# akanimax/thr3ed_atom

Measured on AMD Instinct MI355X. Metric: ray-samples/sec (fwd+bwd) training step, 800x800 images @ 128^3 SH-2 ReLU field, higher is better.
Workload: dtype f32

## Files before the change

thr3ed_atom_amd/csrc/relu_field_kernels.hip:

```cpp
#include <hip/hip_runtime.h>
#include <stdint.h>

#include <atomic>
#include <climits>
#include <cmath>
#include <cstdlib>
#include <type_traits>

#include "relu_field.h"

namespace {

#ifndef RF_FWD_WAVES
#define RF_FWD_WAVES 4
#endif
#ifndef RF_EMIT_WAVES
#define RF_EMIT_WAVES 6
#endif
#ifndef RF_EMIT_G
#define RF_EMIT_G 2
#endif
constexpr int kWave = 64;
constexpr int kWavesPerBlock = 4;
constexpr int kBlock = kWave * kWavesPerBlock;
// ... 1868 lines not shown
  {
    const int4* __restrict__ h4 = reinterpret_cast<const int4*>(hist);
    const int n4 = seg0 >> 2;
    int k4 = t;
    for (; k4 + 3 * 1024 < n4; k4 += 4 * 1024) {
      const int4 a0 = h4[k4], a1 = h4[k4 + 1024], a2 = h4[k4 + 2048], a3 = h4[k4 + 3072];
      front += (a0.x + a0.y) + (a0.z + a0.w) + (a1.x + a1.y) + (a1.z + a1.w) + (a2.x + a2.y) + (a2.z + a2.w) + (a3.x + a3.y) + (a3.z + a3.w);
    }
    for (; k4 < n4; k4 += 1024) {
      const int4 a0 = h4[k4];
      front += (a0.x + a0.y) + (a0.z + a0.w);
    }
  }
#pragma unroll
  for (int d = 1; d < kWave; d <<= 1) front += __shfl_xor(front, d);
  const int k = seg0 + t;
  const int c = k < nkeys ? hist[k] : 0;
  int incl = c;
#pragma unroll
  for (int d = 1; d < kWave; d <<= 1) {
    const int up = __shfl_up(incl, d);
    if (lane >= d) incl += up;
  }
  if (lane == kWave - 1) {
    s_front[wave] = front;
    s_own[wave] = incl;
  }
  __syncthreads();
  int base = 0, before = 0, own = 0;
#pragma unroll
  for (int w = 0; w < 16; ++w) {
    base += s_front[w];
    if (w < wave) before += s_own[w];
    own += s_own[w];
  }
  if (k < nkeys) {
    const int excl = base + before + incl - c;
    offsets[k] = excl;
    cursor[k] = excl;
  }
  if (t == 0 && seg0 + 1024 >= nkeys) offsets[nkeys] = base + own;
}

__global__ __launch_bounds__(1024) void bin_offsets_kernel(BinLists lists, int nkeys) { bin_offsets_body(lists, nkeys, blockIdx.y, blockIdx.x); }

template <int Q>
__global__ __launch_bounds__(256) void scatter_records_kernel(const short* __restrict__ keys, const float4* __restrict__ rec,
                                                              long long capacity, int* __restrict__ cursor,
                                                              float4* __restrict__ out, int* __restrict__ hist, int nkeys) {
  constexpr int NCH = 4;
  __shared__ long long s_slot[4][NCH * kWave];
  __shared__ int s_pos[4][NCH * kWave];
  const int lane = threadIdx.x & (kWave - 1), wave = threadIdx.x >> 6;
  if (hist)
    for (long long k = (long long)blockIdx.x * blockDim.x + threadIdx.x; k < nkeys; k += (long long)gridDim.x * blockDim.x) hist[k] = 0;
  const long long slot0 = ((long long)blockIdx.x * 4 + wave) * (NCH * kWave);
  if (slot0 >= capacity) return;
  int key[NCH], run[NCH], hl[NCH], base[NCH];
  bool head[NCH];
  unsigned long long act[NCH];
#pragma unroll
  for (int i = 0; i < NCH; ++i) {
    const long long slot = slot0 + i * kWave + lane;
    key[i] = slot < capacity ? (int)keys[slot] : -1;
  }
#pragma unroll
  for (int i = 0; i < NCH; ++i) {
    const bool active = key[i] >= 0;
    act[i] = __ballot(active);
    const int prev = __shfl_up(key[i], 1);
    head[i] = active && (lane == 0 || prev != key[i]);
    const unsigned long long heads = __ballot(head[i]);
    const unsigned long long ends = __ballot(head[i] || !active);
    const unsigned long long above = (lane == 63) ? 0ull : (ends & ~((2ull << lane) - 1ull));
    run[i] = (above ? __builtin_ctzll(above) : 64) - lane;
    const unsigned long long below = heads & ((lane == 63) ? ~0ull : ((2ull << lane) - 1ull));
    hl[i] = below ? 63 - __builtin_clzll(below) : 0;
  }
#pragma unroll
  for (int i = 0; i < NCH; ++i) base[i] = head[i] ? atomicAdd(&cursor[key[i]], run[i]) : 0;
  int n_act = 0;
#pragma unroll
  for (int i = 0; i < NCH; ++i) {
    const int pos = __shfl(base[i], hl[i]) + (lane - hl[i]);
    if (key[i] >= 0) {
      const int e = n_act + __popcll(act[i] & ((1ull << lane) - 1ull));
      s_slot[wave][e] = slot0 + i * kWave + lane;
      s_pos[wave][e] = pos;
    }
    n_act += __popcll(act[i]);
  }
  wave_lds_fence();
  const int items = n_act * Q;
  for (int it = lane; it < items; it += kWave) {
    const int e = it / Q, part = it - e * Q;
    out[(long long)s_pos[wave][e] * Q + part] = rec[s_slot[wave][e] * Q + part];
  }
}

constexpr int kBrickThreads = 512;

__host__ __device__ inline int brick_node_stride(int C) { return (C + 3) / 4 * 4; }
__host__ __device__ inline int brick_row_stride(int B, int C) {
  const int row = B * brick_node_stride(C);
  return row + ((48 - row % 64) + 64) % 64;
}
__host__ __device__ inline int brick_slab_stride(int B, int C) {
  const int slab = B * brick_row_stride(B, C);
  return slab + ((8 - slab % 64) + 64) % 64;
}
__host__ __device__ inline int brick_acc_words(int B, int C) { return B * brick_slab_stride(B, C) + 64; }

#ifdef RF_BRICK_PROFILE
__device__ unsigned long long g_brick_prof[8];
#define RF_PROF_MARK(slot)                                                       \
  do {                                                                           \
    const unsigned long long now_ = __builtin_readcyclecounter();                \
    prof_acc_[slot] += now_ - prof_t_;                                           \
    prof_t_ = now_;                                                              \
  } while (0)
#define RF_PROF_START()                                              \
  unsigned long long prof_acc_[8] = {0, 0, 0, 0, 0, 0, 0, 0};        \
  unsigned long long prof_t_ = __builtin_readcyclecounter()
#define RF_PROF_END()                                                            \
  do {                                                                           \
    if (threadIdx.x == 0) {                                                      \
      _Pragma("unroll") for (int s_ = 0; s_ < 8; ++s_)                           \
        if (prof_acc_[s_]) atomicAdd(&g_brick_prof[s_], prof_acc_[s_]);          \
    }                                                                            \
  } while (0)
#else
#define RF_PROF_MARK(slot) do { } while (0)
#define RF_PROF_START() do { } while (0)
#define RF_PROF_END() do { } while (0)
#endif

__device__ __forceinline__ void brick_range_entry(const BrickArgs& a, const long long* __restrict__ offsets, int bx, int by, int bz, int e,
                                                  int& start, int& cnt) {
  const int ex = e / 5, eyz = e - ex * 5;
  const int ox = ex == 2, xf = ex >= 1;
  const int oy = (0x16 >> eyz) & 1, oz = (0x18 >> eyz) & 1;
  const int f0 = (0x32310 >> (4 * eyz)) & 7, f1 = (0x33313 >> (4 * eyz)) & 7;
  const int sx = bx - ox, sy = by - oy, sz = bz - oz;
  start = 0;
  cnt = 0;
  if (sx >= 0 && sy >= 0 && sz >= 0) {
    const long long* off = offsets + ((long long)((((sx << 1) | xf) * a.nby + sy) * a.nbz + sz) << 2);
    const long long rs = off[f0];
    start = (int)rs;
    cnt = (int)(off[f1 + 1] - rs);
  }
}

template <int K, bool ADAM, bool ONE_ROUND, int TH = kBrickThreads, int BX = 8, bool MIRROR = false>
__device__ __forceinline__ void brick_flush(const GridArgs& g, const BrickArgs& a, const float* acc, bool any, int X0, int Y0, int Z0,
                                            float* gdens, float* gfeat) {
  static_assert(!MIRROR || (ADAM && ONE_ROUND && BX == 4), "the mirror write-out rides on the one-round optimizer flush of 4 x 8 x 8 bricks");
  constexpr int C = 3 * K + 1;
  constexpr int CS = (C + 3) / 4 * 4;
  const int B = ONE_ROUND ? 8 : (1 << a.shift);
  const int SY = brick_row_stride(B, C), SX = brick_slab_stride(B, C);
  const int tid = threadIdx.x;
  const bool split = g.layout == RF_LAYOUT_SPLIT;
  if (split && (C & 3) == 0 && (g.dstride & 3) == 0 && (C == 4 || (g.fstride & 3) == 0)) {
    constexpr int QN = C / 4;
    constexpr int QR = QN > 1 ? QN - 1 : 1;
    const int nq = (BX == 4 ? 4 : B) * B * B * QN;
    auto quad_of = [&](int i, int& fx, int& fy, int& fz, int& qd) -> bool {
      const int col = (i >> a.shift) / QN, r = i - col * (B * QN);
      const bool first = r < B;
      fz = first ? r : (r - B) / QR;
      qd = first ? 0 : 1 + (r - B) - fz * QR;
      fx = col >> a.shift;
      fy = col & (B - 1);
      return i < nq && X0 + fx < g.X && Y0 + fy < g.Y && Z0 + fz < g.Z;
    };
    if constexpr (ADAM) {
      constexpr int U = (QN == 7) ? 4 : 1;
      const AdamArgs& ad = a.adam;
      if constexpr (ONE_ROUND) {
        unsigned int bo[QN];
        int lds_at[QN];
        float4 p4[QN];
        vf4 m4[QN], v4[QN];
#pragma unroll
        for (int u = 0; u < QN; ++u) {
          int fx, fy, fz, qd;
          if (u == 0) {
            fx = tid >> 6;
            fy = (tid >> 3) & 7;
            fz = tid & 7;
            qd = 0;
          } else {
            const int j = (u - 1) * TH + tid, col = j / 48, r = j - col * 48;
            fz = r / 6;
            qd = 1 + r - 6 * fz;
            fx = col >> 3;
            fy = col & 7;
          }
          const bool ok = X0 + fx < g.X && Y0 + fy < g.Y && Z0 + fz < g.Z;
          const unsigned int lin = ok ? node_lin(g, X0 + fx, Y0 + fy, Z0 + fz) : 0u;
          const unsigned int o = u == 0 ? __umul24(lin, (unsigned)g.dstride) : __umul24(lin, (unsigned)g.fstride) + 4u * (unsigned)(qd - 1);
          bo[u] = ok ? o * 4u : 0xffffffffu;
          lds_at[u] = fx * SX + fy * SY + fz * CS + 4 * qd;
        }
#pragma unroll
        for (int u = 0; u < QN; ++u) {
          if (bo[u] != 0xffffffffu) {
            const char* pb = reinterpret_cast<const char*>(u == 0 ? ad.p1 : ad.p2);
            const char* mb = reinterpret_cast<const char*>(u == 0 ? ad.m1 : ad.m2);
            const char* vb = reinterpret_cast<const char*>(u == 0 ? ad.v1 : ad.v2);
            p4[u] = *reinterpret_cast<const float4*>(pb + bo[u]);
            m4[u] = __builtin_nontemporal_load(reinterpret_cast<const vf4*>(mb + bo[u]));
            v4[u] = __builtin_nontemporal_load(reinterpret_cast<const vf4*>(vb + bo[u]));
          }
        }
#pragma unroll
        for (int u = 0; u < QN; ++u) {
          if (bo[u] == 0xffffffffu) continue;
          const float4 gq = any ? *reinterpret_cast<const float4*>(&acc[lds_at[u]]) : make_float4(0.f, 0.f, 0.f, 0.f);
          float gg[4] = {gq.x, gq.y, gq.z, gq.w};
          float pn[4] = {p4[u].x, p4[u].y, p4[u].z, p4[u].w};
          if (u == 0 && g.mode == RF_DENSITY_ABS) {
            const float dv = pn[0] * g.rho;
            gg[0] = (dv > 0.f) ? gg[0] : ((dv < 0.f) ? -gg[0] : 0.0f);
          }
          vf4 mn, vn;
#pragma unroll
          for (int c = 0; c < 4; ++c) {
            float mm = m4[u][c], vv = v4[u][c];
            adam_update(pn[c], mm, vv, gg[c], ad.step, ad.b1, ad.b2, ad.eps, ad.inv_bc2_sqrt);
            mn[c] = mm;
            vn[c] = vv;
          }
          char* pb = reinterpret_cast<char*>(u == 0 ? ad.p1 : ad.p2);
          char* mb = reinterpret_cast<char*>(u == 0 ? ad.m1 : ad.m2);
          char* vb = reinterpret_cast<char*>(u == 0 ? ad.v1 : ad.v2);
          *reinterpret_cast<float4*>(pb + bo[u]) = make_float4(pn[0], pn[1], pn[2], pn[3]);
          __builtin_nontemporal_store(mn, reinterpret_cast<vf4*>(mb + bo[u]));
          __builtin_nontemporal_store(vn, reinterpret_cast<vf4*>(vb + bo[u]));
          if constexpr (MIRROR) *reinterpret_cast<float4*>(const_cast<float*>(&acc[lds_at[u]])) = make_float4(pn[0], pn[1], pn[2], pn[3]);
        }
        if constexpr (MIRROR) {
          __syncthreads();
          constexpr int F = 3 * K, FQ = 2 * F, CQ = FQ + 2;
          for (int i = tid; i < 32 * CQ; i += TH) {
            const int col = i / CQ, r = i - col * CQ;
            const int fx = col >> 3, fy = col & 7;
            const float* img = acc + fx * SX + fy * SY;
            const unsigned int lin0 = node_lin(g, X0 + fx, Y0 + fy, Z0);
            float v[4];
            if (r < FQ) {
#pragma unroll
              for (int t = 0; t < 4; ++t) {
                const int e = 4 * r + t;
                const int nz = e / F, f = e - nz * F;
                const int colour = f / K, k = f - colour * K;
                v[t] = img[nz * CS + (k == 0 ? 1 + colour : 4 + colour * (K - 1) + (k - 1))];
              }
              *reinterpret_cast<float4*>(gfeat + (size_t)(__umul24(lin0, (unsigned)F) + 4u * (unsigned)r)) = make_float4(v[0], v[1], v[2], v[3]);
            } else {
              const int z0 = 4 * (r - FQ);
#pragma unroll
              for (int t = 0; t < 4; ++t) v[t] = img[(z0 + t) * CS];
              *reinterpret_cast<float4*>(gdens + (size_t)(lin0 + (unsigned)z0)) = make_float4(v[0], v[1], v[2], v[3]);
            }
          }
        }
        return;
      } else {
      for (int i0 = tid; i0 < nq; i0 += TH * U) {
        unsigned int off[U];
        float4 p4[U];
        vf4 m4[U], v4[U];
#pragma unroll
        for (int u = 0; u < U; ++u) {
          int fx, fy, fz, qd;
          const bool ok = quad_of(i0 + u * TH, fx, fy, fz, qd);
          const unsigned int lin = ok ? node_lin(g, X0 + fx, Y0 + fy, Z0 + fz) : 0u;
          const unsigned int o = qd == 0 ? lin * (unsigned)g.dstride : (lin * (unsigned)g.fstride + 4u * (unsigned)(qd - 1)) | 0x80000000u;
          off[u] = ok ? o : 0xffffffffu;
        }
#pragma unroll
        for (int u = 0; u < U; ++u) {
          if (off[u] != 0xffffffffu) {
            const bool rest = off[u] >> 31;
            const unsigned int o = off[u] & 0x7fffffffu;
#ifdef RF_BRICK_PROFILE
            if (a.stagger & 0x10000) { p4[u] = make_float4(0.f, 0.f, 0.f, 0.f); m4[u] = vf4{0.f, 0.f, 0.f, 0.f}; v4[u] = vf4{1.f, 1.f, 1.f, 1.f}; continue; }
#endif
            p4[u] = *reinterpret_cast<const float4*>((rest ? ad.p2 : ad.p1) + o);
            m4[u] = __builtin_nontemporal_load(reinterpret_cast<const vf4*>((rest ? ad.m2 : ad.m1) + o));
            v4[u] = __builtin_nontemporal_load(reinterpret_cast<const vf4*>((rest ? ad.v2 : ad.v1) + o));
          }
        }
#pragma unroll
        for (int u = 0; u < U; ++u) {
          if (off[u] == 0xffffffffu) continue;
          const bool rest = off[u] >> 31;
          const unsigned int o = off[u] & 0x7fffffffu;
          int fx, fy, fz, qd;
          quad_of(i0 + u * TH, fx, fy, fz, qd);
          const float4 gq = any ? *reinterpret_cast<const float4*>(&acc[fx * SX + fy * SY + fz * CS + 4 * qd]) : make_float4(0.f, 0.f, 0.f, 0.f);
          float gg[4] = {gq.x, gq.y, gq.z, gq.w};
          float pn[4] = {p4[u].x, p4[u].y, p4[u].z, p4[u].w};
          if (!rest && g.mode == RF_DENSITY_ABS) {
// ... 21 lines not shown
          __builtin_nontemporal_store(mn, reinterpret_cast<vf4*>((rest ? ad.m2 : ad.m1) + o));
          __builtin_nontemporal_store(vn, reinterpret_cast<vf4*>((rest ? ad.v2 : ad.v1) + o));
        }
      }
      }
      return;
    }
    for (int i = tid; i < nq; i += TH) {
      int fx, fy, fz, qd;
      if (!quad_of(i, fx, fy, fz, qd)) continue;
      const long long lin = node_lin(g, X0 + fx, Y0 + fy, Z0 + fz);
      float4 v = any ? *reinterpret_cast<const float4*>(&acc[fx * SX + fy * SY + fz * CS + 4 * qd]) : make_float4(0.f, 0.f, 0.f, 0.f);
      if (qd == 0 && g.mode == RF_DENSITY_ABS) {
        const float dv = g.dens[lin * g.dstride] * g.rho;
        v.x = (dv > 0.f) ? v.x : ((dv < 0.f) ? -v.x : 0.0f);
      }
      const long long off = (qd == 0) ? lin * g.dstride : lin * g.fstride + 4 * (qd - 1);
      if (qd == 0) {
        float4* dst = reinterpret_cast<float4*>(gdens + off);
        if (a.accumulate) {
          const float4 o = *dst;
          v = make_float4(o.x + v.x, o.y + v.y, o.z + v.z, o.w + v.w);
        }
        *dst = v;
      } else {
        float4* dst = reinterpret_cast<float4*>(gfeat + off);
        if (a.accumulate) {
          const float4 o = *dst;
          v = make_float4(o.x + v.x, o.y + v.y, o.z + v.z, o.w + v.w);
        }
        const vf4 v4 = {v.x, v.y, v.z, v.w};
        __builtin_nontemporal_store(v4, reinterpret_cast<vf4*>(dst));
      }
    }
    return;
  }
  const int n_first = split ? 4 : 1;
  const int n_second = C - n_first;
  for (int pass = 0; pass < 2; ++pass) {
    const int nch = pass == 0 ? n_first : n_second;
    if (nch == 0) continue;
    const int run = B * nch;
    float* out = pass == 0 ? gdens : gfeat;
    const long long ostride = pass == 0 ? g.dstride : g.fstride;
    for (int i = tid; i < (BX == 4 ? 4 : B) * B * run; i += TH) {
      const int col = i / run, r = i - col * run;
      const int fz = r / nch, c2 = r - fz * nch;
      const int fx = col >> a.shift, fy = col & (B - 1);
      const int X = X0 + fx, Y = Y0 + fy, Z = Z0 + fz;
      if (X >= g.X || Y >= g.Y || Z >= g.Z) continue;
      int lds_c;
      if (split) {
        lds_c = pass * 4 + c2;
      } else if (pass == 0) {
        lds_c = 0;
      } else {
        const int col3 = c2 / K, kk = c2 - col3 * K;
        lds_c = (kk == 0) ? 1 + col3 : 4 + col3 * (K - 1) + (kk - 1);
      }
      const long long lin = node_lin(g, X, Y, Z);
      float v = any ? acc[fx * SX + fy * SY + fz * CS + lds_c] : 0.0f;
      if (lds_c == 0 && g.mode == RF_DENSITY_ABS) {
        const float dv = g.dens[lin * g.dstride] * g.rho;
        v = (dv > 0.f) ? v : ((dv < 0.f) ? -v : 0.0f);
      }
      float* dst = out + lin * ostride + (long long)c2 * (pass == 1 && !split ? a.fmul : 1);
      *dst = a.accumulate ? (*dst + v) : v;
    }
  }
}

__device__ __forceinline__ uint32_t lds_offset(const void* p) { return (uint32_t)(uintptr_t)p; }
template <int OFF>
__device__ __forceinline__ void lds_request_f32(float& v, uint32_t addr) {
  asm volatile("ds_read_b32 %0, %1 offset:%2" : "+v"(v) : "v"(addr), "n"(OFF));
}
__device__ __forceinline__ void lds_request_u8(uint32_t& v, uint32_t addr) {
  asm volatile("ds_read_u8 %0, %1" : "+v"(v) : "v"(addr));
}
__device__ __forceinline__ void lds_wait(uint32_t& a, uint32_t& b) { asm volatile("s_waitcnt lgkmcnt(0)" : "+v"(a), "+v"(b)); }
__device__ __forceinline__ void lds_wait(float& a, float& b, float& c, float& d, uint32_t& f) {
  asm volatile("s_waitcnt lgkmcnt(0)" : "+v"(a), "+v"(b), "+v"(c), "+v"(d), "+v"(f));
}
__device__ __forceinline__ void lds_wait(float& a, float& b, float& c, float& d, float& e, uint32_t& f) {
  asm volatile("s_waitcnt lgkmcnt(0)" : "+v"(a), "+v"(b), "+v"(c), "+v"(d), "+v"(e), "+v"(f));
}
__device__ __forceinline__ void lds_wait(float& a, float& b, float& c, float& d, float& e, float& e2, float& e3, uint32_t& f) {
  asm volatile("s_waitcnt lgkmcnt(0)" : "+v"(a), "+v"(b), "+v"(c), "+v"(d), "+v"(e), "+v"(e2), "+v"(e3), "+v"(f));
}

constexpr int kGatherBatch = 256;
constexpr int kGatherWtab = 24;
__host__ __device__ constexpr int gather_record_words(int C4) { return C4 + 8; }
typedef float f32x4 __attribute__((ext_vector_type(4)));

__host__ __device__ inline int gather_lds_words(int B, int C, int BX = 8) {
  const int C4 = (C + 3) / 4 * 4;
  const int gb = BX == 4 ? kGatherBatch / 2 : kGatherBatch;
  const int batch = gb * gather_record_words(C4) + (gb + 4) * kGatherWtab;
  const int image = BX == 4 ? 4 * brick_slab_stride(B, C) + 64 : brick_acc_words(B, C);
  return batch > image ? batch : image;
}

template <int K, bool ADAM, bool ONE_ROUND = false, bool SPLIT = false, int BX = 8, bool MIRROR = false>
__global__ __launch_bounds__(BX == 4 ? kBrickThreads / 2 : kBrickThreads, (K > 9 ? 2 : 4)) void brick_gather_kernel(GridArgs g, BrickArgs a, float* gdens, float* gfeat) {
  static_assert(BX == 8 || (BX == 4 && ONE_ROUND && !SPLIT), "4 x 8 x 8 bricks: 8-node y and z edges, one workgroup per brick");
  constexpr int TH = BX == 4 ? kBrickThreads / 2 : kBrickThreads;
  constexpr int NWV = TH / 64;
  constexpr int GB = TH / 2;
  constexpr int GROW = GB + 4;
  constexpr int C = 3 * K + 1;
  constexpr int C4 = (C + 3) / 4 * 4;
  constexpr int QW = record_quads(K);
  constexpr int QN = record_quads(1);
  constexpr int NT = (C4 + 15) / 16;
  static_assert(NT == 1 || NT == 2 || NT == 4, "one, two or four 16-channel blocks (SH degree 0 / base lists, 1-2, 3)");
  constexpr int CS = C4;
  constexpr int NW = GB / 64;
  constexpr bool SEP = BX == 4 && K == 9 && ONE_ROUND && !SPLIT;
  extern __shared__ __attribute__((aligned(16))) float acc[];
  float* rows = acc;
  float* wtab = acc + GB * gather_record_words(C4);
  __shared__ uint32_t s_tmask[GB];
  __shared__ unsigned char s_list[4 * NWV][GB + 24];
  __shared__ __attribute__((aligned(16))) int s_wstart[kMaxRangesKind], s_wcum[kMaxRangesKind + 8];
  __shared__ __attribute__((aligned(16))) int s_nstart[kMaxRangesKind], s_ncum[kMaxRangesKind + 8];
  __shared__ int s_part[4];
  constexpr int GBN = SEP ? TH : GB;
  constexpr int BROW = TH + 4;
  constexpr int NWB = TH / 64;
  float* btab = acc;
  float* brows = acc + 20 * BROW;
  unsigned char* bmask = reinterpret_cast<unsigned char*>(s_tmask);
  unsigned char(*blist)[TH + 24] = reinterpret_cast<unsigned char(*)[TH + 24]>(&s_list[0][0]);
  static_assert(!SEP || (20 * BROW + 4 * TH <= GB * gather_record_words(C4) + GROW * kGatherWtab && TH <= kGatherBatch && NWV * (TH + 24) <= 4 * NWV * (GB + 24)),
                "the base-channel batch of the separable form fits the full-width batch's buffers, its indices a byte");
  const int B = ONE_ROUND ? 8 : (1 << a.shift);
  const int bshift = ONE_ROUND ? 3 : a.shift;
  const int SY = brick_row_stride(B, C), SX = brick_slab_stride(B, C);

  RF_PROF_START();
  const int tid = threadIdx.x;
  const int lane = tid & (kWave - 1);
  const int wave = tid >> 6;
  const int parts = SPLIT ? a.parts : 1;
  const int part = SPLIT ? (int)(blockIdx.x % (unsigned)parts) : 0;
  const int brick_local = SPLIT ? (int)(blockIdx.x / (unsigned)parts) : (int)blockIdx.x;
  const int brick = a.brick_first + brick_local;
  auto lists_of = [&](int nl) { return SPLIT ? (nl > part ? (nl - part + parts - 1) / parts : 0) : nl; };
  auto list_index = [&](int ll) { return SPLIT ? part + ll * parts : ll; };
  const int nwide_p = lists_of(a.nwide), nnarrow_p = lists_of(a.nnarrow);
  const int bz = brick % a.nbz, by = (brick / a.nbz) % a.nby, bx = brick / (a.nbz * a.nby);
  const int X0 = bx << (BX == 4 ? 2 : bshift), Y0 = by << bshift, Z0 = bz << bshift;
  {
    const int kind = tid >> 7, i = tid & 127;
    int start = 0, cnt = 0;
    if (tid < 256) {
      const int nl = kind ? nnarrow_p : nwide_p;
      if (i < kRangeEntries * nl) {
        const int l = nl == 1 ? 0 : i / kRangeEntries;
        const int li = list_index(l);
        const long long* offs = (!SPLIT && nl == 1) ? (kind ? a.narrow[0].offsets : a.wide[0].offsets) : (kind ? a.narrow[li].offsets : a.wide[li].offsets);
        brick_range_entry(a, offs, bx, by, bz, i - l * kRangeEntries, start, cnt);
      }
    }
    int cum = cnt;
#pragma unroll
    for (int d = 1; d < kWave; d <<= 1) {
      const int up = __shfl_up(cum, d);
      if (lane >= d) cum += up;
    }
    if (wave < 4 && lane == kWave - 1) s_part[wave] = cum;
    __syncthreads();
    if (tid < 256) {
      if (wave & 1) cum += s_part[wave - 1];
      int* st_ = kind ? s_nstart : s_wstart;
      int* cu_ = kind ? s_ncum : s_wcum;
      if (i < kMaxRangesKind) {
        st_[i] = start;
        cu_[i + 1] = cum;
      }
      if (i == 0) cu_[0] = 0;
    }
    __syncthreads();
  }
  const int total = s_wcum[kMaxRangesKind];
  const int total_d = s_ncum[kMaxRangesKind];
  bool any = total > 0 || total_d > 0;
  if (!SPLIT && !any && a.accumulate) return;
  RF_PROF_MARK(0);

  const int npz = B >> 2, npy = B >> 1;
  const int ntiles = BX == 4 ? 16 : (B * B * B) >> 4;
  const int mi = lane & 15;
  const int mdx = mi >> 3, mdy = (mi >> 2) & 1, mdz = mi & 3;
  const int kk = lane >> 4;
  const int jj = lane & 15;

  f32x4 accr[4][NT];
#pragma unroll
  for (int tl = 0; tl < 4; ++tl)
#pragma unroll
    for (int nt = 0; nt < NT; ++nt) accr[tl][nt] = f32x4{0.f, 0.f, 0.f, 0.f};
  f32x4 naccr = f32x4{0.f, 0.f, 0.f, 0.f};

  if (any) {
    const int nba = (total + GB - 1) / GB, nbd = (total_d + GBN - 1) / GBN;
    uint32_t wprev = 0x00ffffffu;
    const int rec_id = tid & (GB - 1);
    const int half = tid >= GB;

    auto stage = [&](auto expand_tag, float4 q0, float4 q1, float4 q2, int nrec) {
      constexpr bool EXPAND = decltype(expand_tag)::value;
      constexpr int RW = gather_record_words(EXPAND ? C4 : 4);
      if (half == 0) {
        uint32_t tm = 0, wnow = 0x00ffffffu;
        float* wcol = wtab + rec_id;
#pragma unroll
        for (int ax = 0; ax < 3; ++ax) {
          const int c1 = (int)((wprev >> (8 * ax)) & 0xffu);
          if (c1 != 0xff) {
            if (c1 >= 1) wcol[(ax * 8 + c1 - 1) * GROW] = 0.0f;
            if (c1 < (BX == 4 && ax == 0 ? 4 : B)) wcol[(ax * 8 + c1) * GROW] = 0.0f;
          }
        }
        if (rec_id < nrec) {
          const float idx[3] = {q0.x, q0.y, q0.z};
          const int org[3] = {X0, Y0, Z0};
          uint32_t pb[3];
          wnow = 0;
#pragma unroll
          for (int ax = 0; ax < 3; ++ax) {
            const float fl = floorf(idx[ax]);
            const int c = (int)fl - org[ax];
            const int sh = ax == 2 ? 2 : 1;
            uint32_t bits = 0;
            if (c >= 0) {
              wcol[(ax * 8 + c) * GROW] = (fl + 1.0f) - idx[ax];
              bits |= 1u << (c >> sh);
            }
            if (c + 1 < (BX == 4 && ax == 0 ? 4 : B)) {
              wcol[(ax * 8 + c + 1) * GROW] = idx[ax] - fl;
              bits |= 1u << ((c + 1) >> sh);
            }
            pb[ax] = bits;
            wnow |= (uint32_t)(c + 1) << (8 * ax);
          }
          uint32_t yz = 0;
#pragma unroll
          for (int py = 0; py < 4; ++py)
            if ((pb[1] >> py) & 1u) yz |= pb[2] << (py * npz);
#pragma unroll
          for (int px = 0; px < 4; ++px)
            if ((pb[0] >> px) & 1u) tm |= yz << (px * npy * npz);
        }
        wprev = wnow;
        s_tmask[rec_id] = tm;
      }
      float* row = rows + rec_id * RW;
      if constexpr (EXPAND) {
        const float graw[3] = {q1.x, q1.y, q1.z};
        constexpr int NQ = C4 / 4;
        if (half == 0) {
          *reinterpret_cast<float4*>(row) = make_float4(q0.w, graw[0] * kC0, graw[1] * kC0, graw[2] * kC0);
        } else {
          float Y[16];
          sh_basis<K>(q1.w, q2.x, q2.y, Y);
#pragma unroll
          for (int q = 1; q < NQ; ++q) {
            float v[4];
#pragma unroll
            for (int x = 0; x < 4; ++x) v[x] = (4 * q + x < C) ? record_channel<K>(4 * q + x, q0.w, graw, Y) : 0.0f;
            *reinterpret_cast<float4*>(row + 4 * q) = make_float4(v[0], v[1], v[2], v[3]);
          }
        }
      } else {
        if (half == 0) *reinterpret_cast<float4*>(row) = q1;
      }
    };
    auto stage_blocks = [&](float4 q0, float4 q1, int nrec) {
      uint32_t tm = 0, wnow = 0x00ffffffu;
      float* wcol = btab + tid;
      constexpr int first_row[3] = {0, 4, 12}, nodes[3] = {4, 8, 8};
#pragma unroll
      for (int ax = 0; ax < 3; ++ax) {
        const int c1 = (int)((wprev >> (8 * ax)) & 0xffu);
        if (c1 != 0xff) {
          if (c1 >= 1) wcol[(first_row[ax] + c1 - 1) * BROW] = 0.0f;
          if (c1 < nodes[ax]) wcol[(first_row[ax] + c1) * BROW] = 0.0f;
        }
      }
      if (tid < nrec) {
        const float idx[3] = {q0.x, q0.y, q0.z};
        const int org[3] = {X0, Y0, Z0};
        uint32_t pb[3];
        wnow = 0;
#pragma unroll
        for (int ax = 0; ax < 3; ++ax) {
          const float fl = floorf(idx[ax]);
          const int c = (int)fl - org[ax];
          uint32_t bits = 0;
          if (c >= 0) {
            wcol[(first_row[ax] + c) * BROW] = (fl + 1.0f) - idx[ax];
            bits |= 1u << (c >> 2);
          }
          if (c + 1 < nodes[ax]) {
            wcol[(first_row[ax] + c + 1) * BROW] = idx[ax] - fl;
            bits |= 1u << ((c + 1) >> 2);
          }
          pb[ax] = bits;
          wnow |= (uint32_t)(c + 1) << (8 * ax);
        }
        if (pb[0]) tm = ((pb[1] & 1u) ? pb[2] : 0u) | ((pb[1] & 2u) ? pb[2] << 2 : 0u);
      }
      wprev = wnow;
      bmask[tid] = (unsigned char)tm;
      *reinterpret_cast<float4*>(brows + 4 * tid) = q1;
    };
    auto process = [&](auto wide_tag, int nrec) {
      constexpr bool WIDE = decltype(wide_tag)::value;
      constexpr int RW = gather_record_words(WIDE ? C4 : 4);
      constexpr int NTW = WIDE ? NT : 1;
      RF_PROF_MARK(7);
      __syncthreads();
      RF_PROF_MARK(2);
      int cnt[4] = {0, 0, 0, 0};
#if defined(RF_BRICK_PROFILE) || defined(RF_BRICK_ABLATE)
      const bool no_lists = a.stagger & 0x200000, no_tiles = a.stagger & 0x100000;
#else
      constexpr bool no_lists = false, no_tiles = false;
#endif
      if (!no_lists)
#pragma unroll
      for (int wd = 0; wd < NW; ++wd) {
        if (wd * 64 >= nrec) break;
        const uint32_t tmv = s_tmask[wd * 64 + lane] >> wave;
#pragma unroll
        for (int tl = 0; tl < 4; ++tl) {
          const bool hit = (tmv >> (NWV * tl)) & 1u;
          const unsigned long long m = __ballot(hit);
          const int pos = cnt[tl] + __builtin_amdgcn_mbcnt_hi((uint32_t)(m >> 32), __builtin_amdgcn_mbcnt_lo((uint32_t)m, 0));
          if (hit) s_list[(tl * NWV + wave)][pos] = (unsigned char)(wd * 64 + lane);
          cnt[tl] += __popcll(m);
        }
      }
#pragma unroll
      for (int tl = 0; tl < 4; ++tl)
        if (lane < 8) s_list[(tl * NWV + wave)][cnt[tl] + lane] = 0;
#pragma unroll
      for (int tl = 0; tl < 4; ++tl) {
        const int t = (tl * NWV + wave);
        const int n = cnt[tl];
        if (t < ntiles && n > 0 && !no_tiles) {
          const int pz = t % npz, py = (t / npz) % npy, px = t / (npz * npy);
          const float* wx = wtab + (2 * px + mdx) * GROW;
          const float* wy = wtab + (8 + 2 * py + mdy) * GROW;
          const float* wz = wtab + (16 + 4 * pz + mdz) * GROW;
          const float* gbase = rows + (WIDE ? jj : (jj & 3));
          const uint32_t a_list = lds_offset(s_list[t]) + kk;
          const uint32_t a_x = lds_offset(wx), a_y = lds_offset(wy), a_z = lds_offset(wz), a_g = lds_offset(gbase);
          const int nq = (n + 3) >> 2;
          uint32_t ra = 0, rb = 0;
          float aw0 = 0.f, aw1 = 0.f, aw2 = 0.f, bw0 = 0.f, bw1 = 0.f, bw2 = 0.f;
          float ag0 = 0.f, ag1 = 0.f, ag2 = 0.f, ag3 = 0.f, bg0 = 0.f, bg1 = 0.f, bg2 = 0.f, bg3 = 0.f;
          auto request_ops = [&](float& w0, float& w1, float& w2, float& g0, float& g1, float& g2, float& g3, uint32_t r) {
            lds_request_f32<0>(w0, a_x + 4 * r);
            lds_request_f32<0>(w1, a_y + 4 * r);
            lds_request_f32<0>(w2, a_z + 4 * r);
            const uint32_t a_row = a_g + (uint32_t)__umul24(r, RW * 4);
            lds_request_f32<0>(g0, a_row);
            if constexpr (NTW > 1) lds_request_f32<64>(g1, a_row);
            if constexpr (NTW > 2) {
              lds_request_f32<128>(g2, a_row);
              lds_request_f32<192>(g3, a_row);
            }
          };
          auto wait_ops = [&](float& w0, float& w1, float& w2, float& g0, float& g1, float& g2, float& g3, uint32_t& r) {
            if constexpr (NTW > 2)
              lds_wait(w0, w1, w2, g0, g1, g2, g3, r);
            else
              lds_wait(w0, w1, w2, g0, g1, r);
          };
          auto multiply = [&](float w0, float w1, float w2, float g0, float g1, float g2, float g3, int q) {
            const float wv = (w0 * w1) * w2;
            const float wa = (4 * q + kk < n) ? wv : 0.0f;
            const float ga = (WIDE || jj < 4) ? g0 : 0.0f;
            accr[tl][0] = __builtin_amdgcn_mfma_f32_16x16x4f32(wa, ga, accr[tl][0], 0, 0, 0);
            if constexpr (NTW > 1) accr[tl][1] = __builtin_amdgcn_mfma_f32_16x16x4f32(wa, g1, accr[tl][1], 0, 0, 0);
            if constexpr (NTW > 2) {
              accr[tl][2] = __builtin_amdgcn_mfma_f32_16x16x4f32(wa, g2, accr[tl][2], 0, 0, 0);
              accr[tl][3] = __builtin_amdgcn_mfma_f32_16x16x4f32(wa, g3, accr[tl][3], 0, 0, 0);
            }
          };
          lds_request_u8(ra, a_list);
          lds_request_u8(rb, a_list + 4);
          lds_wait(ra, rb);
          request_ops(aw0, aw1, aw2, ag0, ag1, ag2, ag3, ra);
          for (int q = 0; q < nq; q += 2) {
            wait_ops(aw0, aw1, aw2, ag0, ag1, ag2, ag3, rb);
            lds_request_u8(ra, a_list + 4 * q + 8);
            request_ops(bw0, bw1, bw2, bg0, bg1, bg2, bg3, rb);
            multiply(aw0, aw1, aw2, ag0, ag1, ag2, ag3, q);
            if (q + 1 < nq) {
              wait_ops(bw0, bw1, bw2, bg0, bg1, bg2, bg3, ra);
              lds_request_u8(rb, a_list + 4 * q + 12);
              request_ops(aw0, aw1, aw2, ag0, ag1, ag2, ag3, ra);
              multiply(bw0, bw1, bw2, bg0, bg1, bg2, bg3, q + 1);
            }
          }
          wait_ops(aw0, aw1, aw2, ag0, ag1, ag2, ag3, ra);
          wait_ops(bw0, bw1, bw2, bg0, bg1, bg2, bg3, rb);
        }
      }
      RF_PROF_MARK(3);
      __syncthreads();
      RF_PROF_MARK(2);
    };
    auto process_blocks = [&](int nrec) {
      RF_PROF_MARK(7);
      __syncthreads();
      RF_PROF_MARK(2);
#if defined(RF_BRICK_PROFILE) || defined(RF_BRICK_ABLATE)
      const bool no_lists = a.stagger & 0x200000, no_tiles = a.stagger & 0x100000;
#else
      constexpr bool no_lists = false, no_tiles = false;
#endif
      unsigned char* list = blist[wave];
      int n = 0;
      if (!no_lists)
#pragma unroll
        for (int wd = 0; wd < NWB; ++wd) {
          if (wd * 64 >= nrec) break;
          const bool hit = (bmask[wd * 64 + lane] >> wave) & 1u;
          const unsigned long long m = __ballot(hit);
          const int pos = n + __builtin_amdgcn_mbcnt_hi((uint32_t)(m >> 32), __builtin_amdgcn_mbcnt_lo((uint32_t)m, 0));
          if (hit) list[pos] = (unsigned char)(wd * 64 + lane);
          n += __popcll(m);
        }
      if (lane < 8) list[n + lane] = 0;
      if (n > 0 && !no_tiles) {
        const uint32_t a_list = lds_offset(list) + kk;
        const uint32_t a_x = lds_offset(btab + (mi & 3) * BROW);
        const uint32_t a_y = lds_offset(btab + (4 + 4 * (wave >> 1) + (jj >> 2)) * BROW);
        const uint32_t a_z = lds_offset(btab + (12 + 4 * (wave & 1) + (jj & 3)) * BROW);
        const uint32_t a_g = lds_offset(brows + (mi >> 2));
        const int nq = (n + 3) >> 2;
        uint32_t ra = 0, rb = 0;
        float xa = 0.f, ya = 0.f, za = 0.f, ga = 0.f, xb = 0.f, yb = 0.f, zb = 0.f, gb = 0.f;
        auto request_ops = [&](float& wx, float& wy, float& wz, float& g, uint32_t r) {
          lds_request_f32<0>(wx, a_x + 4 * r);
          lds_request_f32<0>(wy, a_y + 4 * r);
          lds_request_f32<0>(wz, a_z + 4 * r);
          lds_request_f32<0>(g, a_g + 16 * r);
        };
        auto multiply = [&](float wx, float wy, float wz, float g, int q) {
          const float av = g * wx;
          const float aa = (4 * q + kk < n) ? av : 0.0f;
          naccr = __builtin_amdgcn_mfma_f32_16x16x4f32(aa, wy * wz, naccr, 0, 0, 0);
        };
        lds_request_u8(ra, a_list);
        lds_request_u8(rb, a_list + 4);
        lds_wait(ra, rb);
        request_ops(xa, ya, za, ga, ra);
        for (int q = 0; q < nq; q += 2) {
          lds_wait(xa, ya, za, ga, rb);
          lds_request_u8(ra, a_list + 4 * q + 8);
          request_ops(xb, yb, zb, gb, rb);
          multiply(xa, ya, za, ga, q);
          if (q + 1 < nq) {
            lds_wait(xb, yb, zb, gb, ra);
            lds_request_u8(rb, a_list + 4 * q + 12);
            request_ops(xa, ya, za, ga, ra);
            multiply(xb, yb, zb, gb, q + 1);
          }
        }
        lds_wait(xa, ya, za, ga, ra);
        lds_wait(xb, yb, zb, gb, rb);
      }
      RF_PROF_MARK(3);
      __syncthreads();
      RF_PROF_MARK(2);
    };
    using Yes = std::integral_constant<bool, true>;
    using No = std::integral_constant<bool, false>;

    int sri = 0, dri = 0;
    int rlo = 0, rhi = 0, dlo = 0, dhi = 0;
    const float4* rptr = a.wide[SPLIT ? min(part, kMaxListsPerKind - 1) : 0].rec;
    const float4* dptr = a.narrow[SPLIT ? min(part, kMaxListsPerKind - 1) : 0].rec;
    float4 w0 = make_float4(0.f, 0.f, 0.f, 0.f), w1 = w0, w2 = w0, d0 = w0, d1 = w0;
    auto range_of = [&](const int* cum, int v, int nlists, int from) -> int {
      if (nlists == 1) {
        const int4* c4 = reinterpret_cast<const int4*>(cum);
        const int4 c0 = c4[0], c1 = c4[1], c2 = c4[2], c3 = c4[3];
        return (c0.y <= v) + (c0.z <= v) + (c0.w <= v) + (c1.x <= v) + (c1.y <= v) + (c1.z <= v) + (c1.w <= v) + (c2.x <= v) + (c2.y <= v) + (c2.z <= v) +
               (c2.w <= v) + (c3.x <= v) + (c3.y <= v) + (c3.z <= v);
      }
      int i = from;
      while (cum[i] > v) --i;
      while (cum[i + 1] <= v) ++i;
      return i;
    };
    auto fetch_wide = [&](int s) {
      const int nrec = min(GB, total - s * GB);
      const int v = s * GB + min(rec_id, nrec - 1);
      if (v < rlo || v >= rhi) {
        sri = range_of(s_wcum, v, nwide_p, sri);
        rlo = s_wcum[sri];
        rhi = s_wcum[sri + 1];
        rptr = ((!SPLIT && a.nwide == 1) ? a.wide[0].rec : a.wide[list_index(sri / kRangeEntries)].rec) + (long long)(s_wstart[sri] - rlo) * QW;
      }
      const float4* p = rptr + (long long)v * QW;
      w0 = load_f4<RF_NT_RECORD_LOAD>(p);
      w1 = load_f4<RF_NT_RECORD_LOAD>(p + 1);
      if constexpr (QW > 2) w2 = load_f4<RF_NT_RECORD_LOAD>(p + 2);
    };
    auto fetch_narrow = [&](int sd) {
      const int nrec = min(GBN, total_d - sd * GBN);
      const int v = sd * GBN + min(SEP ? tid : rec_id, nrec - 1);
      if (v < dlo || v >= dhi) {
        dri = range_of(s_ncum, v, nnarrow_p, dri);
        dlo = s_ncum[dri];
        dhi = s_ncum[dri + 1];
        dptr = ((!SPLIT && a.nnarrow == 1) ? a.narrow[0].rec : a.narrow[list_index(dri / kRangeEntries)].rec) + (long long)(s_nstart[dri] - dlo) * QN;
      }
      const float4* p = dptr + (long long)v * QN;
      d0 = load_f4<RF_NT_RECORD_LOAD>(p);
      d1 = load_f4<RF_NT_RECORD_LOAD>(p + 1);
    };
    if (nbd > 0) fetch_narrow(0);
    if (nba > 0) fetch_wide(0);
    if (!SEP || nba > 0) {
      for (int i = tid; i < GROW * kGatherWtab / 4; i += TH) reinterpret_cast<float4*>(wtab)[i] = make_float4(0.f, 0.f, 0.f, 0.f);
      __syncthreads();
    }
    for (int s = 0; s < nba; ++s) {
      const int nrec = min(GB, total - s * GB);
      if constexpr (K > 1)
        stage(Yes{}, w0, w1, w2, nrec);
      else
        stage(No{}, w0, w1, w2, nrec);
      RF_PROF_MARK(1);
      fetch_wide(min(s + 1, nba - 1));
      RF_PROF_MARK(6);
      process(Yes{}, nrec);
    }
    if constexpr (SEP) {
      if (nbd > 0) {
#pragma unroll
        for (int r = 0; r < 20; ++r) btab[r * BROW + tid] = 0.0f;
        wprev = 0x00ffffffu;
      }
    }
    for (int sd = 0; sd < nbd; ++sd) {
      const int nrec = min(GBN, total_d - sd * GBN);
      if constexpr (SEP)
        stage_blocks(d0, d1, nrec);
      else
        stage(No{}, d0, d1, d1, nrec);
      RF_PROF_MARK(1);
      fetch_narrow(min(sd + 1, nbd - 1));
      RF_PROF_MARK(6);
      if constexpr (SEP)
        process_blocks(nrec);
      else
        process(No{}, nrec);
    }
#pragma unroll
    for (int tl = 0; tl < 4; ++tl) {
      const int t = (tl * NWV + wave);
      if (t < ntiles) {
        const int pz = t % npz, py = (t / npz) % npy, px = t / (npz * npy);
#pragma unroll
        for (int nt = 0; nt < NT; ++nt) {
          const int ch = 16 * nt + jj;
#pragma unroll
          for (int e = 0; e < 4; ++e) {
            const int i = 4 * kk + e;
            const int nx = 2 * px + (i >> 3), ny = 2 * py + ((i >> 2) & 1), nz = 4 * pz + (i & 3);
            if (ch < CS) acc[nx * SX + ny * SY + nz * CS + ch] = accr[tl][nt][e];
          }
        }
      }
    }
    if constexpr (SEP) {
      if (total_d > 0) {
        __syncthreads();
        const int ny = 4 * (wave >> 1) + (jj >> 2), nz = 4 * (wave & 1) + (jj & 3);
#pragma unroll
        for (int e = 0; e < 4; ++e) acc[e * SX + ny * SY + nz * CS + kk] += naccr[e];
      }
    }
    __syncthreads();
    RF_PROF_MARK(5);
  }
  if constexpr (SPLIT) {
    const int words = brick_acc_words(B, C);
    int* state = a.part_state + (long long)brick_local * (1 + parts);
    unsigned long long* images = reinterpret_cast<unsigned long long*>(a.partial + (long long)brick_local * parts * words);
    const int pairs = words / 2;
    __shared__ int s_arrival;
    if (any) {
      unsigned long long* mine = images + (long long)part * pairs;
      const unsigned long long* src = reinterpret_cast<const unsigned long long*>(acc);
      for (int i = tid; i < pairs; i += TH) __hip_atomic_store(mine + i, src[i], __ATOMIC_RELAXED, __HIP_MEMORY_SCOPE_AGENT);
      if (tid == 0) __hip_atomic_store(&state[1 + part], 1, __ATOMIC_RELAXED, __HIP_MEMORY_SCOPE_AGENT);
    }
    asm volatile("s_waitcnt vmcnt(0)" ::: "memory");
    __syncthreads();
    if (tid == 0) s_arrival = __hip_atomic_fetch_add(&state[0], 1, __ATOMIC_RELAXED, __HIP_MEMORY_SCOPE_AGENT);
    __syncthreads();
    if (s_arrival != parts - 1) return;
    for (int j = 0; j < parts; ++j) {
      if (j == part) continue;
      if (__hip_atomic_load(&state[1 + j], __ATOMIC_RELAXED, __HIP_MEMORY_SCOPE_AGENT) == 0) continue;
      const unsigned long long* other = images + (long long)j * pairs;
      float2* own = reinterpret_cast<float2*>(acc);
      for (int i = tid; i < pairs; i += TH) {
        const unsigned long long o = __hip_atomic_load(other + i, __ATOMIC_RELAXED, __HIP_MEMORY_SCOPE_AGENT);
        float2 v = any ? own[i] : make_float2(0.f, 0.f);
        v.x += __uint_as_float((uint32_t)o);
        v.y += __uint_as_float((uint32_t)(o >> 32));
        own[i] = v;
      }
      any = true;
      __syncthreads();
    }
    if (tid <= parts) state[tid] = 0;
    __syncthreads();
  }
#if defined(RF_BRICK_PROFILE) || defined(RF_BRICK_ABLATE)
  if (!(a.stagger & 0x400000))
#endif
  brick_flush<K, ADAM, ONE_ROUND, TH, BX, MIRROR>(g, a, acc, any, X0, Y0, Z0, gdens, gfeat);
  RF_PROF_MARK(4);
  RF_PROF_END();
}

__device__ __forceinline__ long long channel_offset(const GridArgs& g, unsigned int lin, int ch, int K, bool& in_first) {
  if (g.layout == RF_LAYOUT_REFERENCE) {
    in_first = ch == 0;
    if (ch == 0) return (long long)lin * g.dstride;
    if (ch < 4) return (long long)lin * g.fstride + (long long)(ch - 1) * K;
    const int j = ch - 4, colour = j / (K - 1), kk = 1 + j - colour * (K - 1);
    return (long long)lin * g.fstride + (long long)colour * K + kk;
  }
  in_first = ch < 4;
  return ch < 4 ? (long long)lin * g.dstride + ch : (long long)lin * g.fstride + (ch - 4);
}

struct UpsampleAxis {
  int i0, i1;
  float w0, w1;
};
__device__ __forceinline__ UpsampleAxis upsample_axis(int dst, int in_size, float scale) {
  float src = fmaf(scale, (float)dst + 0.5f, -0.5f);
  src = src < 0.0f ? 0.0f : src;
  UpsampleAxis a;
  a.i0 = min((int)floorf(src), in_size - 1);
  a.i1 = a.i0 + (a.i0 < in_size - 1 ? 1 : 0);
  const float lambda = fminf(fmaxf(src - (float)a.i0, 0.0f), 1.0f);
  a.w0 = 1.0f - lambda;
  a.w1 = lambda;
  return a;
}

__global__ void upsample_grid_kernel(GridArgs src, GridArgs dst, float* dst_first, float* dst_second, long long total) {
  const int C = dst.F + 1, K = dst.F / 3;
  const float sx = (float)src.X / (float)dst.X, sy = (float)src.Y / (float)dst.Y, sz = (float)src.Z / (float)dst.Z;
  for (long long it = (long long)blockIdx.x * blockDim.x + threadIdx.x; it < total; it += (long long)gridDim.x * blockDim.x) {
    const int ch = (int)(it % C);
    long long node = it / C;
    const int z = (int)(node % dst.Z);
    node /= dst.Z;
    const int y = (int)(node % dst.Y), x = (int)(node / dst.Y);
    const UpsampleAxis ax = upsample_axis(x, src.X, sx), ay = upsample_axis(y, src.Y, sy), az = upsample_axis(z, src.Z, sz);
    auto at = [&](int xi, int yi, int zi) -> float {
      bool first;
      const long long off = channel_offset(src, node_lin(src, xi, yi, zi), ch, K, first);
      return (first ? src.dens : src.feat)[off];
    };
    float val[8], wgt[8];
#pragma unroll
    for (int k = 0; k < 8; ++k) {
      const int dx = k >> 2, dy = (k >> 1) & 1, dz = k & 1;
      val[k] = at(dx ? ax.i1 : ax.i0, dy ? ay.i1 : ay.i0, dz ? az.i1 : az.i0);
      wgt[k] = ((dx ? ax.w1 : ax.w0) * (dy ? ay.w1 : ay.w0)) * (dz ? az.w1 : az.w0);
    }
    int uc;
    if (ch == 0) {
      uc = dst.F;
    } else if (ch < 4) {
      uc = (ch - 1) * K;
    } else {
      const int j = ch - 4, colour = j / (K - 1);
      uc = colour * K + 1 + (j - colour * (K - 1));
    }
    float v;
    if (uc < (C & ~7)) {
      v = fmaf(val[7], wgt[7], val[6] * wgt[6]);
#pragma unroll
      for (int k = 5; k >= 0; --k) v = fmaf(val[k], wgt[k], v);
    } else {
      v = fmaf(val[0], wgt[0], val[1] * wgt[1]);
#pragma unroll
      for (int k = 2; k < 8; ++k) v = fmaf(val[k], wgt[k], v);
    }
    bool first;
    const long long off = channel_offset(dst, node_lin(dst, x, y, z), ch, K, first);
    (first ? dst_first : dst_second)[off] = v;
  }
}
// ... 2829 lines not shown
```

Measured before the change: 16.90 billion.

## Prefetch two wide record batches up front and split records across thread pairs

In the separable brick gather path, the first two wide-record batches are now loaded before the weight-table clear, so both global fetches overlap it. Each thread now loads only two of the three record quads, selected by 'half', which cuts per-thread load registers. An optional path that computes brick ranges per thread from uniform offsets is also added but left disabled by default. The added register pressure from the extra prefetch buffers could lower occupancy.

```diff
diff --git a/thr3ed_atom_amd/csrc/relu_field_kernels.hip b/thr3ed_atom_amd/csrc/relu_field_kernels.hip
--- a/thr3ed_atom_amd/csrc/relu_field_kernels.hip
+++ b/thr3ed_atom_amd/csrc/relu_field_kernels.hip
@@ -2044,6 +2044,67 @@
   }
 }
 
+#ifndef RF_BRICK_SCALAR_RANGES
+#define RF_BRICK_SCALAR_RANGES 0
+#endif
+#ifndef RF_BRICK_TOP_PREFETCH
+#define RF_BRICK_TOP_PREFETCH 1
+#endif
+#ifndef RF_BRICK_TWO_QUADS
+#define RF_BRICK_TWO_QUADS 1
+#endif
+
+struct BrickRangePick {
+  int lo, hi, base;
+};
+
+template <int NP>
+__device__ __forceinline__ int brick_ranges_uniform(const BrickArgs& a, const long long* __restrict__ offsets, bool have, int bx, int by, int bz,
+                                                    int tid, int* s_start, int* s_cum, const int (&u)[NP], BrickRangePick (&pick)[NP]) {
+  int st[kRangeEntries], cu[kRangeEntries + 1], rs[kRangeEntries], re[kRangeEntries];
+#pragma unroll
+  for (int e = 0; e < kRangeEntries; ++e) {
+    const int ex = e / 5, eyz = e - ex * 5;
+    const int ox = ex == 2, xf = ex >= 1;
+    const int oy = (0x16 >> eyz) & 1, oz = (0x18 >> eyz) & 1;
+    const int f0 = (0x32310 >> (4 * eyz)) & 7, f1 = (0x33313 >> (4 * eyz)) & 7;
+    const int sx = max(bx - ox, 0), sy = max(by - oy, 0), sz = max(bz - oz, 0);
+    const long long* off = offsets + ((long long)((((sx << 1) | xf) * a.nby + sy) * a.nbz + sz) << 2);
+    rs[e] = (int)off[f0];
+    re[e] = (int)off[f1 + 1];
+  }
+  __builtin_amdgcn_sched_barrier(0);
+  cu[0] = 0;
+#pragma unroll
+  for (int e = 0; e < kRangeEntries; ++e) {
+    const int ex = e / 5, eyz = e - ex * 5;
+    const bool ok = have && bx - (ex == 2) >= 0 && by - ((0x16 >> eyz) & 1) >= 0 && bz - ((0x18 >> eyz) & 1) >= 0;
+    st[e] = ok ? rs[e] : 0;
+    cu[e + 1] = cu[e] + (ok ? re[e] - rs[e] : 0);
+  }
+#pragma unroll
+  for (int p = 0; p < NP; ++p) pick[p] = BrickRangePick{0, 0, 0};
+  int ms = 0, mc = 0;
+#pragma unroll
+  for (int e = 0; e < kRangeEntries; ++e) {
+    if (tid == e) {
+      ms = st[e];
+      mc = cu[e];
+    }
+    if (cu[e + 1] > cu[e]) {
+#pragma unroll
+      for (int p = 0; p < NP; ++p)
+        if (cu[e] <= u[p]) pick[p] = BrickRangePick{cu[e], cu[e + 1], st[e] - cu[e]};
+    }
+  }
+  if (tid == kRangeEntries) mc = cu[kRangeEntries];
+  if (tid <= kRangeEntries) {
+    if (tid < kRangeEntries) s_start[tid] = ms;
+    s_cum[tid] = mc;
+  }
+  return cu[kRangeEntries];
+}
+
 template <int K, bool ADAM, bool ONE_ROUND, int TH = kBrickThreads, int BX = 8, bool MIRROR = false>
 __device__ __forceinline__ void brick_flush(const GridArgs& g, const BrickArgs& a, const float* acc, bool any, int X0, int Y0, int Z0,
                                             float* gdens, float* gfeat) {
@@ -2371,7 +2432,17 @@
   const int nwide_p = lists_of(a.nwide), nnarrow_p = lists_of(a.nnarrow);
   const int bz = brick % a.nbz, by = (brick / a.nbz) % a.nby, bx = brick / (a.nbz * a.nby);
   const int X0 = bx << (BX == 4 ? 2 : bshift), Y0 = by << bshift, Z0 = bz << bshift;
-  {
+  constexpr bool TOP = SEP && RF_BRICK_TOP_PREFETCH;
+  constexpr bool TQ = SEP && RF_BRICK_TWO_QUADS;
+  const bool one_list = SEP && RF_BRICK_SCALAR_RANGES && a.nwide <= 1 && a.nnarrow <= 1 && a.nwide + a.nnarrow >= 1;
+  BrickRangePick wpick[2] = {}, npick[1] = {};
+  int total = 0, total_d = 0;
+  if (one_list) {
+    const int uw[2] = {tid & (GB - 1), GB + (tid & (GB - 1))};
+    total = brick_ranges_uniform<2>(a, a.nwide == 1 ? a.wide[0].offsets : a.narrow[0].offsets, a.nwide == 1, bx, by, bz, tid, s_wstart, s_wcum, uw, wpick);
+    const int un[1] = {tid};
+    total_d = brick_ranges_uniform<1>(a, a.nnarrow == 1 ? a.narrow[0].offsets : a.wide[0].offsets, a.nnarrow == 1, bx, by, bz, tid, s_nstart, s_ncum, un, npick);
+  } else {
     const int kind = tid >> 7, i = tid & 127;
     int start = 0, cnt = 0;
     if (tid < 256) {
@@ -2402,9 +2473,9 @@
       if (i == 0) cu_[0] = 0;
     }
     __syncthreads();
-  }
-  const int total = s_wcum[kMaxRangesKind];
-  const int total_d = s_ncum[kMaxRangesKind];
+    total = s_wcum[kMaxRangesKind];
+    total_d = s_ncum[kMaxRangesKind];
+  }
   bool any = total > 0 || total_d > 0;
   if (!SPLIT && !any && a.accumulate) return;
   RF_PROF_MARK(0);
@@ -2707,7 +2778,12 @@
     int rlo = 0, rhi = 0, dlo = 0, dhi = 0;
     const float4* rptr = a.wide[SPLIT ? min(part, kMaxListsPerKind - 1) : 0].rec;
     const float4* dptr = a.narrow[SPLIT ? min(part, kMaxListsPerKind - 1) : 0].rec;
-    float4 w0 = make_float4(0.f, 0.f, 0.f, 0.f), w1 = w0, w2 = w0, d0 = w0, d1 = w0;
+    f32x4 w0, w1, w2, d0, d1;
+    f32x4 x0, x1, x2;
+    if constexpr (!SEP) w0 = w1 = w2 = d0 = d1 = f32x4{0.f, 0.f, 0.f, 0.f};
+    auto as_vec = [](float4 q) { return f32x4{q.x, q.y, q.z, q.w}; };
+    auto as_f4 = [](f32x4 q) { return make_float4(q[0], q[1], q[2], q[3]); };
+    static_assert(!TQ || QW == 3, "two quads per thread: compact three-quad records");
     auto range_of = [&](const int* cum, int v, int nlists, int from) -> int {
       if (nlists == 1) {
         const int4* c4 = reinterpret_cast<const int4*>(cum);
@@ -2720,7 +2796,7 @@
       while (cum[i + 1] <= v) ++i;
       return i;
     };
-    auto fetch_wide = [&](int s) {
+    auto locate_wide = [&](int s) -> const float4* {
       const int nrec = min(GB, total - s * GB);
       const int v = s * GB + min(rec_id, nrec - 1);
       if (v < rlo || v >= rhi) {
@@ -2729,12 +2805,20 @@
         rhi = s_wcum[sri + 1];
         rptr = ((!SPLIT && a.nwide == 1) ? a.wide[0].rec : a.wide[list_index(sri / kRangeEntries)].rec) + (long long)(s_wstart[sri] - rlo) * QW;
       }
-      const float4* p = rptr + (long long)v * QW;
-      w0 = load_f4<RF_NT_RECORD_LOAD>(p);
-      w1 = load_f4<RF_NT_RECORD_LOAD>(p + 1);
-      if constexpr (QW > 2) w2 = load_f4<RF_NT_RECORD_LOAD>(p + 2);
+      return rptr + (long long)v * QW;
     };
-    auto fetch_narrow = [&](int sd) {
+    auto load_wide = [&](const float4* p, f32x4& q0, f32x4& q1, f32x4& q2) {
+      if constexpr (TQ) {
+        q0 = as_vec(load_f4<RF_NT_RECORD_LOAD>(p + half));
+        q1 = as_vec(load_f4<RF_NT_RECORD_LOAD>(p + half + 1));
+      } else {
+        q0 = as_vec(load_f4<RF_NT_RECORD_LOAD>(p));
+        q1 = as_vec(load_f4<RF_NT_RECORD_LOAD>(p + 1));
+        if constexpr (QW > 2) q2 = as_vec(load_f4<RF_NT_RECORD_LOAD>(p + 2));
+      }
+    };
+    auto fetch_wide = [&](int s, f32x4& q0, f32x4& q1, f32x4& q2) { load_wide(locate_wide(s), q0, q1, q2); };
+    auto locate_narrow = [&](int sd) -> const float4* {
       const int nrec = min(GBN, total_d - sd * GBN);
       const int v = sd * GBN + min(SEP ? tid : rec_id, nrec - 1);
       if (v < dlo || v >= dhi) {
@@ -2743,24 +2827,89 @@
         dhi = s_ncum[dri + 1];
         dptr = ((!SPLIT && a.nnarrow == 1) ? a.narrow[0].rec : a.narrow[list_index(dri / kRangeEntries)].rec) + (long long)(s_nstart[dri] - dlo) * QN;
       }
-      const float4* p = dptr + (long long)v * QN;
-      d0 = load_f4<RF_NT_RECORD_LOAD>(p);
-      d1 = load_f4<RF_NT_RECORD_LOAD>(p + 1);
+      return dptr + (long long)v * QN;
     };
-    if (nbd > 0) fetch_narrow(0);
-    if (nba > 0) fetch_wide(0);
+    auto load_narrow = [&](const float4* p) {
+      d0 = as_vec(load_f4<RF_NT_RECORD_LOAD>(p));
+      d1 = as_vec(load_f4<RF_NT_RECORD_LOAD>(p + 1));
+    };
+    auto fetch_narrow = [&](int sd) { load_narrow(locate_narrow(sd)); };
+    auto pin = [&](f32x4& q) { asm volatile("" : "+v"(q)); };
+    auto stage_wide = [&](f32x4& v0, f32x4& v1, f32x4& v2, int nrec) {
+      if constexpr (SEP) {
+        pin(v0);
+        pin(v1);
+        if constexpr (!TQ) pin(v2);
+      }
+      const float4 q0 = as_f4(v0), q1 = as_f4(v1), q2 = as_f4(v2);
+      if constexpr (TQ) {
+        if (half == 0)
+          stage(Yes{}, q0, q1, q1, nrec);
+        else
+          stage(Yes{}, q0, q0, q1, nrec);
+      } else if constexpr (K > 1) {
+        stage(Yes{}, q0, q1, q2, nrec);
+      } else {
+        stage(No{}, q0, q1, q2, nrec);
+      }
+    };
+    if constexpr (SEP) {
+      const float4 *pa = rptr, *pb = rptr, *pd = dptr;
+      if (one_list) {
+        rlo = wpick[TOP ? 1 : 0].lo;
+        rhi = wpick[TOP ? 1 : 0].hi;
+        rptr = a.wide[0].rec + (long long)wpick[TOP ? 1 : 0].base * QW;
+        pa = a.wide[0].rec + ((long long)wpick[0].base + min(rec_id, total - 1)) * QW;
+        pb = a.wide[0].rec + ((long long)wpick[1].base + min(GB + rec_id, total - 1)) * QW;
+        dlo = npick[0].lo;
+        dhi = npick[0].hi;
+        dptr = a.narrow[0].rec + (long long)npick[0].base * QN;
+        pd = dptr + (long long)min(tid, total_d - 1) * QN;
+      } else {
+        if (nbd > 0) pd = locate_narrow(0);
+        if (nba > 0) {
+          pa = locate_wide(0);
+          if constexpr (TOP) pb = locate_wide(min(1, nba - 1));
+        }
+      }
+      if (nba > 0) {
+        load_wide(pa, w0, w1, w2);
+        if constexpr (TOP) load_wide(pb, x0, x1, x2);
+      }
+      if (nbd > 0) load_narrow(pd);
+    } else {
+      if (nbd > 0) fetch_narrow(0);
+      if (nba > 0) fetch_wide(0, w0, w1, w2);
+    }
     if (!SEP || nba > 0) {
       for (int i = tid; i < GROW * kGatherWtab / 4; i += TH) reinterpret_cast<float4*>(wtab)[i] = make_float4(0.f, 0.f, 0.f, 0.f);
       __syncthreads();
-    }
-    for (int s = 0; s < nba; ++s) {
+    } else if (one_list) {
+      __syncthreads();
+    }
+    int s_first = 0;
+    if constexpr (TOP) {
+      if (nba > 0) {
+        const int nrec0 = min(GB, total);
+        stage_wide(w0, w1, w2, nrec0);
+        RF_PROF_MARK(1);
+        process(Yes{}, nrec0);
+        if (nba > 1) {
+          const int nrec1 = min(GB, total - GB);
+          stage_wide(x0, x1, x2, nrec1);
+          RF_PROF_MARK(1);
+          fetch_wide(min(2, nba - 1), w0, w1, w2);
+          RF_PROF_MARK(6);
+          process(Yes{}, nrec1);
+        }
+      }
+      s_first = 2;
+    }
+    for (int s = s_first; s < nba; ++s) {
       const int nrec = min(GB, total - s * GB);
-      if constexpr (K > 1)
-        stage(Yes{}, w0, w1, w2, nrec);
-      else
-        stage(No{}, w0, w1, w2, nrec);
+      stage_wide(w0, w1, w2, nrec);
       RF_PROF_MARK(1);
-      fetch_wide(min(s + 1, nba - 1));
+      fetch_wide(min(s + 1, nba - 1), w0, w1, w2);
       RF_PROF_MARK(6);
       process(Yes{}, nrec);
     }
@@ -2773,10 +2922,13 @@
     }
     for (int sd = 0; sd < nbd; ++sd) {
       const int nrec = min(GBN, total_d - sd * GBN);
-      if constexpr (SEP)
-        stage_blocks(d0, d1, nrec);
-      else
-        stage(No{}, d0, d1, d1, nrec);
+      if constexpr (SEP) {
+        pin(d0);
+        pin(d1);
+        stage_blocks(as_f4(d0), as_f4(d1), nrec);
+      } else {
+        stage(No{}, as_f4(d0), as_f4(d1), as_f4(d1), nrec);
+      }
       RF_PROF_MARK(1);
       fetch_narrow(min(sd + 1, nbd - 1));
       RF_PROF_MARK(6);
```

New measurement: 17.04 billion (median of 6 runs). Within noise of the previous version (+0.8%).
